# MicroYY/VoxelHashing

Hardware: AMD Instinct MI355X
Metric: depth frames/sec integrate+raycast @640x480, 4 cm voxel; HBM GB/s vs peak (higher is better)
Workload: dtype f32

## Files before the change

### include/vh_api.h

```cpp
#ifndef VH_API_H
#define VH_API_H

#include "vh_types.h"

#ifdef __cplusplus
extern "C" {
#endif

typedef void* vhStream_t;

const char* vh_version(void);
const char* vh_error_string(int code);
const char* vh_last_error_message(void);

int vh_malloc(void** devPtr, size_t bytes);
int vh_free(void* devPtr);
int vh_malloc_host(void** hostPtr, size_t bytes);
int vh_free_host(void* hostPtr);
int vh_memcpy_h2d(void* dst, const void* src, size_t bytes, vhStream_t stream);
int vh_memcpy_d2h(void* dst, const void* src, size_t bytes, vhStream_t stream);
int vh_memset(void* dst, int value, size_t bytes, vhStream_t stream);
int vh_time_next_launch(void* startEvent, void* stopEvent);
int vh_time_launch_after(uint32_t skip, void* startEvent, void* stopEvent);
int vh_stream_create(vhStream_t* out);
// ... 68 lines not shown
int vh_stream_in_device(const VhHashData* hd, const VhHashParams* hp, uint32_t n, const VhSDFBlockDesc* d_descs, const VhVoxel* d_blocks,
                        int32_t lockToken, uint32_t* d_failed, uint32_t* d_bitMask, uint32_t chunkBit, uint32_t* d_mapped, uint32_t tag,
                        vhStream_t stream);
int vh_stream_in_pass1(const VhHashData* hd, const VhHashParams* hp, uint32_t n, uint32_t heapCountPrev,
                       const VhSDFBlockDesc* d_descs, int32_t lockToken, vhStream_t stream);
int vh_stream_in_pass2(const VhHashData* hd, const VhHashParams* hp, uint32_t n, uint32_t heapCountPrev,
                       const VhSDFBlockDesc* d_descs, const VhVoxel* d_blocks, vhStream_t stream);

int vh_synth_frame(const double* h_spheres, int nSpheres, int inside, const float camToWorld[16],
                   const VhDepthCameraParams* cp, float* d_depth, float* d_color4, vhStream_t stream);
enum { VH_OP_ALLOC = 0, VH_OP_DELETE = 1, VH_OP_INSERT = 2, VH_OP_LOOKUP = 3, VH_OP_NEW_PASS = 4 };
int vh_debug_hash_ops(const VhHashData* hd, const VhHashParams* hp, const int32_t* d_ops, int32_t* d_results,
                      uint32_t n, vhStream_t stream);

int vh_debug_check_fast_math(float divisor, uint32_t modulus, uint32_t n, uint32_t seed, uint32_t* d_mismatches, vhStream_t stream);

int vh_debug_check_refined_division(uint32_t n, uint32_t seed, uint32_t* d_mismatches, vhStream_t stream);
int vh_debug_check_weighted_colour(uint32_t* d_out, vhStream_t stream);
int vh_debug_valu_probe(uint32_t mode, uint32_t wavesPerSimd, uint32_t iters, uint32_t* d_stamps, uint32_t* numWaves, vhStream_t stream);

typedef struct VhSceneRep VhSceneRep;
typedef struct VhRayCast VhRayCast;
typedef struct VhChunkGrid VhChunkGrid;

int vh_scene_rep_create(const VhHashParams* hp, const VhSceneOptions* opt, vhStream_t stream, VhSceneRep** out);
void vh_scene_rep_destroy(VhSceneRep* s);
int vh_scene_rep_integrate(VhSceneRep* s, const float rigidTransform[16], const VhDepthCameraData* cam,
                           const VhDepthCameraParams* cp, const uint32_t* d_bitMask);
int vh_scene_rep_set_last_rigid_transform_and_compactify(VhSceneRep* s, const float rigidTransform[16],
                                                         const VhDepthCameraParams* cp);
// ... 309 lines not shown
```

### voxelhashing_amd/csrc/vh_device.hpp

```cpp
#pragma once

#include <hip/hip_runtime.h>
#include <stdint.h>

#include "../../include/vh_types.h"

namespace vhd {

struct F3 { float x, y, z; };
struct I3 { int x, y, z; };

#define VHD __device__ __forceinline__

VHD float minf() { return __int_as_float((int)0xff800000u); }
VHD float pinf() { return __int_as_float((int)0x7f800000u); }

VHD F3 mk3(float x, float y, float z) { F3 r; r.x = x; r.y = y; r.z = z; return r; }
VHD I3 mki3(int x, int y, int z) { I3 r; r.x = x; r.y = y; r.z = z; return r; }
VHD float dot3(F3 a, F3 b) { return a.x * b.x + a.y * b.y + a.z * b.z; }

VHD int f2i(float v) { return __float2int_rz(v); }
VHD uint8_t f2uc(float v) { return (uint8_t)__float2int_rz(fminf(fmaxf(v, 0.0f), 255.0f)); }

VHD int signi(float v) { return (0.0f < v) - (v < 0.0f); }
// ... 477 lines not shown
    const uint32_t a = v0.cw & 0x00ffffffu, c = v1.cw & 0x00ffffffu;
    uint32_t rgb = (a | c) - (((a ^ c) >> 1) & 0x7f7f7f7fu);
    float w0 = (float)v0.weight(), w1 = (float)v1.weight();
    if (hp.m_colorIntegration != VH_COLOR_RUNNING_AVERAGE) rgb = weighted_colour(v0.cw, v1.cw, w0 + w1, 1.0f / (w0 + w1));
    out.sdf = (v0.sdf * w0 + v1.sdf * w1) / (w0 + w1);
    uint32_t w = min(hp.m_integrationWeightMax, v0.weight() + v1.weight());
    out.cw = rgb | ((w & 0xffu) << 24);
    return out;
}


constexpr int kWave = 64;
VHD uint32_t lane_id() { return threadIdx.x & (kWave - 1); }
VHD uint64_t lanemask_lt() { return (1ull << lane_id()) - 1ull; }

inline uint32_t cdiv(uint64_t a, uint64_t b) { return (uint32_t)((a + b - 1) / b); }
inline uint32_t image_tiles(uint32_t width, uint32_t height) { return cdiv(width, 8) * cdiv(height, 8); }

VHD float4 f4_scale(float a, float4 v) { return make_float4(a * v.x, a * v.y, a * v.z, a * v.w); }
VHD float4 f4_add(float4 a, float4 b) { return make_float4(a.x + b.x, a.y + b.y, a.z + b.z, a.w + b.w); }
VHD float4 f4_div(float4 a, float b) { return make_float4(a.x / b, a.y / b, a.z / b, a.w / b); }

template <class Fetch>
VHD float4 bilinear_float4_taps(float x, float y, Fetch fetch, uint32_t W, uint32_t H)
{
    const int px = (int)floorf(x), py = (int)floorf(y);
    const float alpha = x - (float)px, beta = y - (float)py;
    const float mi = minf();
    float4 s0 = make_float4(0.f, 0.f, 0.f, 0.f), s1 = s0;
    float w0 = 0.0f, w1 = 0.0f;
// ... 24 lines not shown
```

### voxelhashing_amd/csrc/vh_kernels.hip

```cpp
#include <hip/hip_runtime.h>

#include <atomic>
#include <cmath>
#include <cstdint>
#include <cstring>

#include "../../include/vh_api.h"
#include "vh_device.hpp"
#include "vh_host_util.hpp"

using namespace vhd;

#include "vh_frame_alloc.hpp"
#include "vh_frame_compactify.hpp"
#include "vh_frame_integrate.hpp"
#include "vh_frame_splat.hpp"

namespace {


struct BlockCache {
    int bx0, by0, bz0, p0;
    int bx1, by1, bz1, p1;
    bool v0, v1;
// ... 18 lines not shown
    else if (!((word >> (h & 31)) & 1u)) p = VH_FREE_ENTRY;
    else p = lookup_ptr(hd, hp, mki3(bx, by, bz));
    bc.bx1 = bc.bx0; bc.by1 = bc.by0; bc.bz1 = bc.bz0; bc.p1 = bc.p0; bc.v1 = bc.v0;
    bc.bx0 = bx; bc.by0 = by; bc.bz0 = bz; bc.p0 = p; bc.v0 = true;
    return p;
}

constexpr int kPtrUnknown = -3;

struct HashLookup {
    const VhHashData& hd;
    const VhHashParams& hp;
    HashMod hm;
    BlockCache bc;
    static constexpr bool kOffsets32 = false;
    VHD int find(int bx, int by, int bz) { return cached_lookup(hd, hp, hm, bc, bx, by, bz); }
    VHD bool first_tap(int bx, int by, int bz, int& handle)
    {
        handle = kPtrUnknown;
        return bucket_maybe_occupied(hd, hash_pos_fast(hm, mki3(bx, by, bz)));
    }
    VHD bool resolve(int, int bxa, int bya, int bza, int bxb, int byb, int bzb, uint32_t straddle, int (&p)[8])
    {
        const int p0 = find(bxa, bya, bza);
        if (p0 == VH_FREE_ENTRY) return false;
#pragma unroll
        for (int j = 0; j < 8; j++) p[j] = p0;
        if (straddle) {
            uint32_t need = 0xfeu;
#pragma unroll
// ... 16 lines not shown
            }
        }
        return true;
    }
};

constexpr uint32_t kTileSlotWords = 12;

template <uint32_t kTileTabSlots, bool OFFSETS32>
struct TileLookup {
    const int* tab;
    bool complete;
    const VhHashData& hd;
    const VhHashParams& hp;
    static constexpr bool kOffsets32 = OFFSETS32;
    VHD static uint32_t slot_of(int bx, int by, int bz)
    {
        return ((__umul24((uint32_t)bx, 0x9E3779u) + __umul24((uint32_t)by, 0x7F4A7Du) + __umul24((uint32_t)bz, 0x85EBCBu)) >> 10) & (kTileTabSlots - 1u);
    }
    VHD static int slot_find(const int* tab, int bx, int by, int bz)
    {
        uint32_t h = slot_of(bx, by, bz);
        for (;;) {
            const int4 e = *reinterpret_cast<const int4*>(&tab[h * kTileSlotWords]);
            if (e.w == VH_FREE_ENTRY) return -1;
            if ((int)(e.x == bx) & (int)(e.y == by) & (int)(e.z == bz)) return (int)h;
            h = (h + 1u) & (kTileTabSlots - 1u);
        }
    }
    VHD int find_any(int bx, int by, int bz) const
// ... 28 lines not shown
#pragma unroll 1
        for (uint32_t j = 0; j < 8u; j++) {
            const int pj = find_any((j & 1u) ? bxb : bxa, (j & 2u) ? byb : bya, (j & 4u) ? bzb : bza);
            if (pj == VH_FREE_ENTRY) return false;
#pragma unroll
            for (uint32_t k = 0; k < 8u; k++) p[k] = (k == j) ? pj : p[k];
        }
        return true;
    }
};

template <uint32_t kTileTabSlots, bool OFFSETS32>
struct TileLookupComplete {
    const int* tab;
    static constexpr bool kOffsets32 = OFFSETS32;
    VHD bool first_tap(int bx, int by, int bz, int& handle) const
    {
        handle = TileLookup<kTileTabSlots, OFFSETS32>::slot_find(tab, bx, by, bz);
        if (handle >= 0) return true;
        handle = kPtrUnknown;
        return false;
    }
    VHD bool resolve(int handle, int bxa, int bya, int bza, int, int, int, uint32_t straddle, int (&p)[8]) const
    {
        const int sl = handle >= 0 ? handle : TileLookup<kTileTabSlots, OFFSETS32>::slot_find(tab, bxa, bya, bza);
        if (sl < 0) return false;
        const int* e = &tab[(uint32_t)sl * kTileSlotWords + 3u];
        int all = 0;
#pragma unroll
        for (uint32_t j = 0; j < 8u; j++) {
// ... 191 lines not shown
{
    RayQ rq;
    rq.cam = cam; rq.dir = dir;
    rq.vs = voxel;
    rq.rvs = 1.0f / rq.vs;
    rq.halfVoxel = rq.vs / 2.0f;
    rq.camq = mk3(cam.x * rq.rvs, cam.y * rq.rvs, cam.z * rq.rvs);
    rq.dirq = mk3(dir.x * rq.rvs, dir.y * rq.rvs, dir.z * rq.rvs);
    const float Q = 1.0f + (fabsf(rq.camq.x) + fabsf(rq.camq.y) + fabsf(rq.camq.z)) +
                    tFar * (fabsf(rq.dirq.x) + fabsf(rq.dirq.y) + fabsf(rq.dirq.z));
    const float margin = Q * (16.0f / 16777216.0f);
    rq.certLim = (Q < 65536.0f) ? 0.5f - margin : -1.0f;
    return rq;
}

struct Bisected {
    float alpha;
    uint32_t color;
    bool accepted;
};
template <class LK>
VHD Bisected bisect(LK& lk, const VhHashData& hd, const RayQ& rq, float lastAlpha, float lastSdf, float t, float dist,
                    float thresSampleDist, float thresDist, uint32_t& cost)
{
    float a = lastAlpha, aDist = lastSdf, b = t, bDist = dist, c = 0.0f;
    uint32_t color = 0u;
    bool success = true;
#pragma unroll 1
    for (int i = 0; i < 3; i++) {
        cost += kCostSample;
        c = a + (aDist / (aDist - bDist)) * (b - a);
        Taps ctp;
        tap_coords(rq, c, ctp);
        float cDist = 0.0f;
        if (!trilinear<true>(hd, rq.vs, lk, kPtrUnknown, ctp, mk3(rq.cam.x + c * rq.dir.x, rq.cam.y + c * rq.dir.y, rq.cam.z + c * rq.dir.z), rq.rvs, cDist, color)) { success = false; break; }
        if (aDist * cDist > 0.0f) { a = c; aDist = cDist; }
        else { b = c; bDist = cDist; }
    }
    Bisected r;
    r.alpha = c;
    r.color = color;
    r.accepted = success && fabsf(lastSdf - dist) < thresSampleDist && fabsf(dist) < thresDist;
    return r;
}

#ifndef VH_PIPELINE_SMALL
#define VH_PIPELINE_SMALL 0
#endif

struct RayHit {
    float alpha;
    uint32_t color;
    bool hit;
// ... 29 lines not shown

    const float tSkip = depthToRayLength * tileZmin;
    float tStop = fminf(rayEnd, depthToRayLength * tileZmax);
#pragma unroll 1
    while (rcur < tSkip && rcur < rayEnd) rcur += inc;
    if (half != 0u) {
        const float tMid = depthToRayLength * zMid;
        if (half == 1u) {
            tStop = fminf(tStop, tMid);
        } else {
#pragma unroll 1
            for (;;) {
                const float nxt = rcur + inc;
                if (!(nxt < tMid) || !(nxt < rayEnd)) break;
                rcur = nxt;
            }
        }
    }

    if constexpr (PIPELINED) {
        struct Pending {
            float r;
            int skipped;
            int state;
            TapLoads L;
        };
        auto fetch = [&](float r0) -> Pending {
            Pending f;
            f.skipped = 0;
            float r = r0;
// ... 100 lines not shown
#endif
            if (ok & (lastValid != 0) & (lastSdf > 0.0f) & (dist < 0.0f)) { candidate = true; break; }
            lastSdf = ok ? dist : lastSdf;
            lastAlpha = ok ? rcur : lastAlpha;
            lastValid = ok ? 1 : 0;
            rcur += inc;
        }
        if (!candidate) break;

        float a = lastAlpha, aDist = lastSdf, b = rcur, bDist = dist, c = 0.0f;
        uint32_t color2 = 0u;
        bool success = true;
#ifdef VH_RENDER_STATS
        const long long tC0 = clock64();
#endif
#pragma unroll 1
        for (int i = 0; i < 3; i++) {
#ifdef VH_RENDER_STATS
            statTri += 1.0f;
            statIter += 1.0f / (float)__popcll(__ballot(1));
#endif
            cost += kCostSample;
            c = a + (aDist / (aDist - bDist)) * (b - a);
            Taps ctp;
            tap_coords(rq, c, ctp);
            const F3 cpos = mk3(worldCamPos.x + c * worldDir.x, worldCamPos.y + c * worldDir.y, worldCamPos.z + c * worldDir.z);
            float cDist = 0.0f;
            if (!trilinear<true>(hd, rq.vs, lk, kPtrUnknown, ctp, cpos, rq.rvs, cDist, color2)) { success = false; break; }
            if (aDist * cDist > 0.0f) { a = c; aDist = cDist; }
            else { b = c; bDist = cDist; }
        }
#ifdef VH_RENDER_STATS
        statCyc[2] += (float)(clock64() - tC0);
#endif
        if (success && fabsf(lastSdf - dist) < rp.m_thresSampleDist && fabsf(dist) < rp.m_thresDist) {
            out.hit = true;
            out.alpha = c;
            out.color = color2;
            if (GRADIENTS) {
                const F3 iso = mk3(worldCamPos.x + c * worldDir.x, worldCamPos.y + c * worldDir.y, worldCamPos.z + c * worldDir.z);
                const F3 g = gradient_for_point(hd, hp, iso);
                out.normal = mat_mul_d(rp.m_viewMatrix, mk3(-g.x, -g.y, -g.z));
            }
            break;
        }
        lastSdf = dist;
        lastAlpha = rcur;
        lastValid = 1;
        rcur += inc;
    }
}

VHD void store_ray(const VhRayCastData& rd, const VhDepthCameraParams& cp, size_t pix, uint32_t x, uint32_t y, const RayHit& r, bool gradients)
{
    const float mi = minf();
    float depth = mi;
    float4 depth4 = make_float4(mi, mi, mi, mi), normal = depth4, color = depth4;
    if (r.hit) {
        depth = r.alpha / r.depthToRayLength;
        const F3 sk = depth_to_skeleton(cp, x, y, depth);
        depth4 = make_float4(sk.x, sk.y, sk.z, 1.0f);
        color = make_float4((float)(r.color & 0xffu) / 255.f, (float)((r.color >> 8) & 0xffu) / 255.f, (float)((r.color >> 16) & 0xffu) / 255.f, 1.0f);
        if (gradients) normal = make_float4(r.normal.x, r.normal.y, r.normal.z, 1.0f);
    }
    rd.d_depth[pix] = depth;
    reinterpret_cast<float4*>(rd.d_depth4)[pix] = depth4;
    if (rd.d_normals) reinterpret_cast<float4*>(rd.d_normals)[pix] = normal;
    reinterpret_cast<float4*>(rd.d_colors)[pix] = color;
}

#ifdef VH_RENDER_STATS
#define VH_STAT_DECL const long long statT0 = clock64(); const long long statR0 = wall_clock64(); float statTri = 0.0f, statIter = 0.0f; float statCyc[3] = { 0.0f, 0.0f, 0.0f };
#define VH_STAT_ARGS , statTri, statIter, statCyc
#define VH_STAT_STORE                                                                                                                   \
    {                                                                                                                                   \
        const uint32_t hwid = __builtin_amdgcn_s_getreg((31 << 11) | 4), xcc = __builtin_amdgcn_s_getreg((31 << 11) | 20);              \
        reinterpret_cast<float4*>(rd.d_depth4)[pix] = make_float4(statCyc[0], statCyc[1], statCyc[2], 0.0f);                             \
// ... 166 lines not shown
}

template <bool GRADIENTS, uint32_t CAP, bool OFFSETS32>
VHD void render_tile(const VhHashData& hd, const VhHashParams& hp, const VhRayCastData& rd, const VhDepthCameraParams& cp, const VhRayCastParams& rp,
                     uint4* heads, const int4* lists, uint32_t cap, uint32_t* sched, uint32_t phase,
                     int (*tileTab)[2u * CAP * 12u])
{
    constexpr uint32_t kTileTabSlots = 2u * CAP;
    typedef TileLookup<kTileTabSlots, OFFSETS32> Lookup;
    typedef TileLookupComplete<kTileTabSlots, OFFSETS32> LookupComplete;
    static_assert(kTileSlotWords == 12u, "tileTab row size");
    const uint32_t lane = lane_id();
    const uint32_t W = rp.m_width, H = rp.m_height;
    const uint32_t tilesX = (W + 7) / 8, tilesY = (H + 7) / 8;
    const uint32_t nTiles = tilesX * tilesY;
    const uint32_t waveIdx = (uint32_t)__builtin_amdgcn_readfirstlane((int)(blockIdx.x * (blockDim.x / kWave) + (threadIdx.x / kWave)));
    uint32_t tile = waveIdx, half = 0u;
    if (sched && sched[0] == phase) {
        const uint2 e = reinterpret_cast<const uint2*>(sched + 4 + 4u * ((nTiles + 3u) / 4u))[waveIdx];
        tile = e.y == phase ? (e.x & 0xffffffu) : nTiles;
        half = e.y == phase ? (e.x >> 24) : 0u;
    }
    if (tile >= nTiles) return;
#if defined(VH_KNOCKOUT) && VH_KNOCKOUT == 41
    const uint32_t stamp0 = (uint32_t)__builtin_amdgcn_s_memrealtime();
    uint32_t stamp1 = 0u;
    uint4* const stampAt = reinterpret_cast<uint4*>(hd.d_hashCompactified) + (hp.m_hashNumBuckets * VH_HASH_BUCKET_SIZE) / 2u + 3u * waveIdx;
    uint32_t stampList = 0u;
#define VH_WAVE_STAMP(COST)                                                                                                                     \
    if (lane == 0) {                                                                                                                             \
        stampAt[0] = make_uint4(stamp0, stamp1, (uint32_t)__builtin_amdgcn_s_memrealtime(), tile | (half << 24));                               \
        stampAt[1] = make_uint4((COST), __builtin_amdgcn_s_getreg((31 << 11) | 4), __builtin_amdgcn_s_getreg((31 << 11) | 20), 0x57410000u | waveIdx); \
        stampAt[2] = make_uint4(stampList, 0u, 0u, 0u);                                                                                           \
    }
#else
#define VH_WAVE_STAMP(COST)
// ... 86 lines not shown
                if (lane + k * kWave < listed) {
                    const int b3[3] = { mine[k].x, mine[k].y, mine[k].z };
                    float a = vm[11], b = vm[11];
#pragma unroll
                    for (int ax = 0; ax < 3; ax++) {
                        const float lo = (float)(b3[ax] * VH_SDF_BLOCK_SIZE) * vs - growLo, hi = (float)(b3[ax] * VH_SDF_BLOCK_SIZE + VH_SDF_BLOCK_SIZE) * vs + growHi;
                        const float p = vm[8 + ax] * lo, q = vm[8 + ax] * hi;
                        a += fminf(p, q);
                        b += fmaxf(p, q);
                    }
                    const float zs = 2e-3f * fmaxf(fabsf(a), fabsf(b)) + 0.5f * vs;
                    zlo = fminf(zlo, a - zs);
                    zhi = fmaxf(zhi, b + zs);
                }
            }
#pragma unroll
            for (int off = 32; off > 0; off >>= 1) {
                zlo = fminf(zlo, __shfl_xor(zlo, off));
                zhi = fmaxf(zhi, __shfl_xor(zhi, off));
            }
            if (!complete) {
                zlo = fminf(zlo, __uint_as_float(head.x));
                zhi = fmaxf(zhi, __uint_as_float(head.y));
            }
            tileZmin = fmaxf(zlo, 0.0f);
            tileZmax = zhi;
        }
    }
    tileZmin = __int_as_float(__builtin_amdgcn_readfirstlane(__float_as_int(tileZmin)));
    tileZmax = __int_as_float(__builtin_amdgcn_readfirstlane(__float_as_int(tileZmax)));
#if defined(VH_KNOCKOUT) && VH_KNOCKOUT == 41
    stamp1 = (uint32_t)__builtin_amdgcn_s_memrealtime();
#endif
    const uint32_t tileX = (tile % tilesX) * 8, tileY = (tile / tilesX) * 8;
    VH_STAT_DECL
    RayHit out;
    out.hit = false;
    uint32_t cost = 0u;
    if (const uint32_t x = tileX + (lane & 7), y = tileY + (lane >> 3); x < W && y < H && tileZmin <= tileZmax) {
        constexpr bool kPipelined = (CAP > (uint32_t)VH_TILE_LIST_CAPACITY) || VH_PIPELINE_SMALL;
        if (complete) {
            LookupComplete lk{ tab };
            march_ray<GRADIENTS, kPipelined>(lk, hd, hp, cp, rp, x, y, tileZmin, tileZmax, half, 0.5f * (tileZmin + tileZmax), out, cost VH_STAT_ARGS);
        } else {
            Lookup lk{ tab, false, hd, hp };
            march_ray<GRADIENTS, kPipelined>(lk, hd, hp, cp, rp, x, y, tileZmin, tileZmax, half, 0.5f * (tileZmin + tileZmax), out, cost VH_STAT_ARGS);
        }
    }
#pragma unroll
    for (int off = 32; off > 0; off >>= 1) cost = max(cost, (uint32_t)__shfl_xor((int)cost, off));
    const uint32_t laneAfter = lane_id_again();
    const uint32_t x = tileX + (laneAfter & 7), y = tileY + (laneAfter >> 3);
    const bool inImage = x < W && y < H;
    const size_t pix = (size_t)y * W + x;
    if (half != 0u) {
        int* mine = tab;
        int* other = tileTab[waveInGroup ^ 1u];
        if (half == 2u) {
            mine[laneAfter * 8u + 0u] = out.hit ? 1 : 0;
            mine[laneAfter * 8u + 1u] = __float_as_int(out.alpha);
            mine[laneAfter * 8u + 2u] = (int)out.color;
            if (GRADIENTS) { mine[laneAfter * 8u + 3u] = __float_as_int(out.normal.x); mine[laneAfter * 8u + 4u] = __float_as_int(out.normal.y); mine[laneAfter * 8u + 5u] = __float_as_int(out.normal.z); }
            if (laneAfter == 0) mine[64u * 8u] = (int)cost;
        }
        __syncthreads();
        if (half == 2u) { VH_WAVE_STAMP(cost) return; }
        if (!out.hit && other[laneAfter * 8u + 0u] != 0) {
            out.hit = true;
            out.alpha = __int_as_float(other[laneAfter * 8u + 1u]);
            out.color = (uint32_t)other[laneAfter * 8u + 2u];
            if (GRADIENTS) out.normal = mk3(__int_as_float(other[laneAfter * 8u + 3u]), __int_as_float(other[laneAfter * 8u + 4u]), __int_as_float(other[laneAfter * 8u + 5u]));
        }
        cost += (uint32_t)other[64u * 8u];
        if (laneAfter == 0) heads[tile] = make_uint4(0x7f800000u, 0u, 0u, 0u);
    }
    if (inImage) {
        store_ray(rd, cp, pix, x, y, out, GRADIENTS);
        VH_STAT_STORE
    }
    VH_WAVE_STAMP(cost)
    if (sched && laneAfter == 0) sched[4 + tile] = min(cost / kCostClassWidth, kCostClasses - 1u);
}
#undef VH_WAVE_STAMP
#undef VH_STAT_DECL
#undef VH_STAT_ARGS
#undef VH_STAT_STORE

struct CoAlloc {
    VhHashData hd;
    VhHashParams hp;
    VhDepthCameraData cam;
    VhDepthCameraParams cp;
    const uint32_t* bitMask;
    uint2* packed;
    HashMod hm;
    int32_t lockToken;
    uint32_t firstGroup;
};

VHD bool co_alloc(const CoAlloc& job)
{
    if (job.firstGroup == 0u || blockIdx.x < job.firstGroup) return false;
    const uint32_t g = blockIdx.x - job.firstGroup;
    if (g == 0u && threadIdx.x == 0) job.hd.d_hashCompactifiedCounter[0] = 0;
    alloc_tile(job.hd, job.hp, job.cam, job.cp, job.bitMask, job.lockToken, job.hm, job.packed, g * (256u / kWave) + (threadIdx.x / kWave));
    return true;
}
inline uint32_t co_alloc_groups(uint32_t tiles) { return cdiv(tiles, 256u / kWave); }

#ifndef VH_RENDER_WAVES
#define VH_RENDER_WAVES 6
#endif
template <bool GRADIENTS, bool OFFSETS32>
__global__ __launch_bounds__(256) __attribute__((amdgpu_waves_per_eu(VH_RENDER_WAVES, VH_RENDER_WAVES)))
void k_render(VhHashData hd, VhHashParams hp, VhRayCastData rd, VhDepthCameraParams cp, VhRayCastParams rp,
              uint4* heads, const int4* lists, uint32_t cap, uint32_t* sched, uint32_t phase, CoAlloc job)
{
    __shared__ int tileTab[256 / kWave][2u * VH_TILE_LIST_CAPACITY * kTileSlotWords];
    if (co_alloc(job)) return;
    render_tile<GRADIENTS, VH_TILE_LIST_CAPACITY, OFFSETS32>(hd, hp, rd, cp, rp, heads, lists, cap, sched, phase, tileTab);
}

template <bool GRADIENTS, bool OFFSETS32>
__global__ __launch_bounds__(256)
void k_render_large(VhHashData hd, VhHashParams hp, VhRayCastData rd, VhDepthCameraParams cp, VhRayCastParams rp,
                    uint4* heads, const int4* lists, uint32_t cap, uint32_t* sched, uint32_t phase, CoAlloc job)
{
    __shared__ int tileTab[256 / kWave][2u * VH_TILE_LIST_CAPACITY_LARGE * kTileSlotWords];
    if (co_alloc(job)) return;
    render_tile<GRADIENTS, VH_TILE_LIST_CAPACITY_LARGE, OFFSETS32>(hd, hp, rd, cp, rp, heads, lists, cap, sched, phase, tileTab);
}

}

#include "vh_frame_normals.hpp"
#include "vh_frame_checks.hpp"


static uint32_t device_num_cus()
{
    static int numCUs = 0;
    if (numCUs == 0) {
        int dev = 0;
        if (hipGetDevice(&dev) != hipSuccess || hipDeviceGetAttribute(&numCUs, hipDeviceAttributeMultiprocessorCount, dev) != hipSuccess || numCUs <= 0)
// ... 181 lines not shown

uint32_t vh_debug_render_force_offsets64(uint32_t on) { return (uint32_t)g_forceOffsets64.exchange(on ? 1 : 0, std::memory_order_relaxed); }

int vh_render_intervals_co(const VhHashData* hd, const VhHashParams* hp, const VhRayCastData* rd, const VhDepthCameraParams* cp,
                           const VhRayCastParams* rp, uint32_t* d_tileHeads, const VhTileBlock* d_tileBlocks, uint32_t tileCapacity,
                           uint32_t* d_schedule, uint32_t phase, VhFrameJob* fj, vhStream_t stream)
{
    if (!hd || !hp || !rd || !cp || !rp || !rd->d_depth || !d_tileHeads) return VH_ERR_BAD_ARGUMENT;
    const uint32_t tiles = image_tiles(rp->m_width, rp->m_height);
    if (tiles == 0) return VH_OK;
    uint4* h = reinterpret_cast<uint4*>(d_tileHeads);
    const int4* l = reinterpret_cast<const int4*>(d_tileBlocks);
    const uint32_t cap = d_tileBlocks ? tileCapacity : 0u;
    const bool large = cap > (uint32_t)VH_TILE_LIST_CAPACITY;
    uint32_t groups = cdiv(tiles + (d_schedule ? split_tiles(tiles) : 0u), 4);
    CoAlloc job;
    std::memset(&job, 0, sizeof(job));
    if (fj && !fj->allocLaunched && fj->cam.d_depthData && fj->hashData.d_hash && fj->hashParams.m_hashNumBuckets >= 2) {
        job.hd = fj->hashData; job.hp = fj->hashParams; job.cam = fj->cam; job.cp = fj->cp;
        job.bitMask = fj->d_bitMask;
        job.packed = reinterpret_cast<uint2*>(fj->d_packedFrame);
        job.hm = make_hash_mod(fj->hashParams.m_hashNumBuckets);
        job.lockToken = fj->lockToken;
        job.firstGroup = groups;
        groups += co_alloc_groups(image_tiles(fj->cp.m_imageWidth, fj->cp.m_imageHeight));
        fj->allocLaunched = 1;
    }
    const dim3 grid(groups);
    hipStream_t st = (hipStream_t)stream;
    const bool o32 = vh_render_offsets32(hp->m_numSDFBlocks) != 0;
// ... 132 lines not shown
```

### voxelhashing_amd/csrc/vh_util.hip

```cpp
#include <hip/hip_runtime.h>

#include "../../include/vh_api.h"
#include "vh_device.hpp"
#include "vh_host_util.hpp"

using namespace vhd;

namespace {

struct SynthArgs {
    double spheres[4 * 8];
    int nSpheres;
    int inside;
    float T[16];
};

__global__ __launch_bounds__(256) void k_synth(SynthArgs a, VhDepthCameraParams cp, float* depth, float4* color)
{
    const uint32_t idx = blockIdx.x * blockDim.x + threadIdx.x;
    if (idx >= cp.m_imageWidth * cp.m_imageHeight) return;
    const uint32_t u = idx % cp.m_imageWidth, v = idx / cp.m_imageWidth;
    const double ox = (double)a.T[3], oy = (double)a.T[7], oz = (double)a.T[11];
    const double dx = ((double)u - (double)cp.mx) / (double)cp.fx;
    const double dy = ((double)v - (double)cp.my) / (double)cp.fy;
// ... 36 lines not shown
    s ^= s >> 15; s *= 2246822519u; s ^= s >> 13; s *= 3266489917u; s ^= s >> 16;
    uint32_t u = s * 747796405u + 2891336453u;
    float a;
    if ((i & 7u) == 7u) {
        a = __uint_as_float(u);
        const uint32_t ex = (u >> 23) & 0xffu;
        if (ex == 0xffu || ex < 0x10u || ex > 0xe8u) a = (float)(int)u * 1.0e-6f;
    } else {
        a = ((float)(int)u) * (1.0f / 2147483648.0f) * (((i >> 3) & 1u) ? 400.0f : 8.0f);
    }
    const float rb = 1.0f / b;
    const float q0 = a / b, q1 = div_exact(a, b, rb);
    if (__float_as_uint(q0) != __float_as_uint(q1) && !(q0 == 0.0f && q1 == 0.0f)) atomicAdd(&mismatches[0], 1u);
    if ((s % hm.d) != umod_fast(s, hm)) atomicAdd(&mismatches[1], 1u);
    if ((u % hm.d) != umod_fast(u, hm)) atomicAdd(&mismatches[1], 1u);
    if (i < 64u) {
        const uint32_t e = 0xffffffffu - i;
        if ((e % hm.d) != umod_fast(e, hm)) atomicAdd(&mismatches[1], 1u);
        if ((i % hm.d) != umod_fast(i, hm)) atomicAdd(&mismatches[1], 1u);
    }
}

}

extern "C" {

int vh_synth_frame(const double* h_spheres, int nSpheres, int inside, const float camToWorld[16],
                   const VhDepthCameraParams* cp, float* d_depth, float* d_color4, vhStream_t stream)
{
    if (!h_spheres || !camToWorld || !cp || !d_depth || !d_color4 || nSpheres < 0 || nSpheres > 8) return VH_ERR_BAD_ARGUMENT;
    SynthArgs a;
    for (int i = 0; i < 4 * nSpheres; i++) a.spheres[i] = h_spheres[i];
    a.nSpheres = nSpheres;
    a.inside = inside;
    for (int i = 0; i < 16; i++) a.T[i] = camToWorld[i];
    const uint64_t n = (uint64_t)cp->m_imageWidth * cp->m_imageHeight;
    if (n == 0) return VH_OK;
    k_synth<<<cdiv(n, 256), 256, 0, (hipStream_t)stream>>>(a, *cp, d_depth, reinterpret_cast<float4*>(d_color4));
    return vh_last_launch_error();
}

int vh_debug_check_fast_math(float divisor, uint32_t modulus, uint32_t n, uint32_t seed, uint32_t* d_mismatches, vhStream_t stream)
{
    if (!d_mismatches || modulus < 2 || !(divisor > 0.0f)) return VH_ERR_BAD_ARGUMENT;
    VH_HIP(hipMemsetAsync(d_mismatches, 0, 2 * sizeof(uint32_t), (hipStream_t)stream));
    if (n == 0) return VH_OK;
    k_check_fast_math<<<cdiv(n, 256), 256, 0, (hipStream_t)stream>>>(divisor, make_hash_mod(modulus), n, seed, d_mismatches);
    return vh_last_launch_error();
}

}
```

### voxelhashing_amd/lib.py

```python
import ctypes as C
import os

import numpy as np

from . import vhtypes as T

_HERE = os.path.dirname(os.path.abspath(__file__))
LIB_PATH = os.environ.get("VH_LIB_PATH") or os.path.join(_HERE, "libvoxelhashing_amd.so")
_LIB = None

P = C.POINTER
_F16 = P(C.c_float)
_VP = C.c_void_p

PROTOTYPES = {
    "vh_version": (C.c_char_p, []),
    "vh_error_string": (C.c_char_p, [C.c_int]),
    "vh_last_error_message": (C.c_char_p, []),
    "vh_malloc": (C.c_int, [P(_VP), C.c_size_t]),
    "vh_free": (C.c_int, [_VP]),
    "vh_malloc_host": (C.c_int, [P(_VP), C.c_size_t]),
    "vh_free_host": (C.c_int, [_VP]),
    "vh_memcpy_h2d": (C.c_int, [_VP, _VP, C.c_size_t, _VP]),
    "vh_memcpy_d2h": (C.c_int, [_VP, _VP, C.c_size_t, _VP]),
# ... 30 lines not shown
    "vh_debug_render_force_offsets64": (C.c_uint32, [C.c_uint32]),
    "vh_compute_normals": (C.c_int, [_VP, _VP, C.c_uint32, C.c_uint32, _VP]),
    "vh_render_intervals_co": (C.c_int, [P(T.HashData), P(T.HashParams), P(T.RayCastData), P(T.DepthCameraParams), P(T.RayCastParams), _VP, _VP, C.c_uint32, _VP, C.c_uint32, P(T.FrameJob), _VP]),
    "vh_compute_normals_co": (C.c_int, [_VP, _VP, C.c_uint32, C.c_uint32, P(T.FrameJob), _VP]),
    "vh_compute_normals_co2": (C.c_int, [_VP, _VP, C.c_uint32, C.c_uint32, P(T.FrameJob), P(T.RayCastParams), _VP, _VP, C.c_uint32, _VP, C.c_uint32, _VP, _VP]),
    "vh_stream_out_pass1": (C.c_int, [P(T.HashData), P(T.HashParams), C.c_uint32, C.c_uint32, C.c_float, _F16, _VP, _VP, C.c_uint32, C.c_int32, _VP]),
    "vh_stream_out_pass2": (C.c_int, [P(T.HashData), P(T.HashParams), _VP, _VP, C.c_uint32, _VP]),
    "vh_stream_out_device": (C.c_int, [P(T.HashData), P(T.HashParams), C.c_uint32, C.c_uint32, C.c_float, _F16, _VP, _VP, _VP, C.c_uint32, C.c_int32, _VP, _VP]),
    "vh_publish_count": (C.c_int, [_VP, _VP, C.c_uint32, _VP]),
    "vh_stream_in_device": (C.c_int, [P(T.HashData), P(T.HashParams), C.c_uint32, _VP, _VP, C.c_int32, _VP, _VP, C.c_uint32, _VP, C.c_uint32, _VP]),
    "vh_stream_in_pass1": (C.c_int, [P(T.HashData), P(T.HashParams), C.c_uint32, C.c_uint32, _VP, C.c_int32, _VP]),
    "vh_stream_in_pass2": (C.c_int, [P(T.HashData), P(T.HashParams), C.c_uint32, C.c_uint32, _VP, _VP, _VP]),
    "vh_synth_frame": (C.c_int, [_VP, C.c_int, C.c_int, _F16, P(T.DepthCameraParams), _VP, _VP, _VP]),
    "vh_debug_hash_ops": (C.c_int, [P(T.HashData), P(T.HashParams), _VP, _VP, C.c_uint32, _VP]),
    "vh_debug_check_fast_math": (C.c_int, [C.c_float, C.c_uint32, C.c_uint32, C.c_uint32, _VP, _VP]),
    "vh_debug_valu_probe": (C.c_int, [C.c_uint32, C.c_uint32, C.c_uint32, _VP, P(C.c_uint32), _VP]),
    "vh_debug_check_refined_division": (C.c_int, [C.c_uint32, C.c_uint32, _VP, _VP]),
    "vh_debug_check_weighted_colour": (C.c_int, [_VP, _VP]),
    "vh_publish_words": (C.c_int, [_VP, _VP, _VP, C.c_uint32, _VP]),
    "vh_stream_out_probe": (C.c_int, [_VP, _VP, C.c_uint32, C.c_uint32, C.c_float, _VP, _VP, _VP, C.c_uint32, _VP]),
    "vh_scene_rep_create": (C.c_int, [P(T.HashParams), P(T.SceneOptions), _VP, P(_VP)]),
    "vh_scene_rep_destroy": (None, [_VP]),
    "vh_scene_rep_integrate": (C.c_int, [_VP, _F16, P(T.DepthCameraData), P(T.DepthCameraParams), _VP]),
    "vh_scene_rep_set_last_rigid_transform_and_compactify": (C.c_int, [_VP, _F16, P(T.DepthCameraParams)]),
    "vh_scene_rep_reset": (C.c_int, [_VP]),
    "vh_scene_rep_get_hash_data": (C.c_int, [_VP, P(T.HashData)]),
    "vh_scene_rep_get_hash_params": (C.c_int, [_VP, P(T.HashParams)]),
    "vh_scene_rep_get_heap_free_count": (C.c_int, [_VP, P(C.c_uint32)]),
    "vh_scene_rep_get_num_occupied_blocks": (C.c_int, [_VP, P(C.c_uint32)]),
    "vh_scene_rep_debug_hash": (C.c_int, [_VP, P(C.c_uint32)]),
# ... 322 lines not shown
```

Before: 21980.

## Use DPP wave reductions, colourless bisection steps, and per-lane split-ray costs in raycast

Replaces shuffle-based wave min/max reductions with inline DPP assembly plus readlane, and skips colour fetches in the first two bisection steps when gradients are off. It also changes the split-tile cost accounting to per-lane (reducing after merging halves), adjusts the cost estimate for complete tile lookups, and replaces the colour divide with div_exact. Schedule loading now uses a single 64-bit read and falls back to the wave index when the schedule is stale, and a bounds check on the schedule buffer plus a debug reduce kernel are added. The aim is to cut shuffle/LDS traffic and memory reads in the raycast hot path. In exchange it brings in hand-written asm with hazard nops and changes the scheduling semantics.

```diff
diff --git a/include/vh_api.h b/include/vh_api.h
--- a/include/vh_api.h
+++ b/include/vh_api.h
@@ -106,6 +106,8 @@
                       uint32_t n, vhStream_t stream);
 
 int vh_debug_check_fast_math(float divisor, uint32_t modulus, uint32_t n, uint32_t seed, uint32_t* d_mismatches, vhStream_t stream);
+
+int vh_debug_wave_reduce(const uint32_t* d_in64, uint32_t* d_out192, vhStream_t stream);
 
 int vh_debug_check_refined_division(uint32_t n, uint32_t seed, uint32_t* d_mismatches, vhStream_t stream);
 int vh_debug_check_weighted_colour(uint32_t* d_out, vhStream_t stream);
diff --git a/voxelhashing_amd/csrc/vh_device.hpp b/voxelhashing_amd/csrc/vh_device.hpp
--- a/voxelhashing_amd/csrc/vh_device.hpp
+++ b/voxelhashing_amd/csrc/vh_device.hpp
@@ -515,6 +515,32 @@
 VHD uint32_t lane_id() { return threadIdx.x & (kWave - 1); }
 VHD uint64_t lanemask_lt() { return (1ull << lane_id()) - 1ull; }
 
+#define VH_WAVE_REDUCE(OP, CONSTRAINT)                                                                        \
+    {                                                                                                         \
+        asm("s_nop 1\n\t" OP " %0, %0, %0 row_shr:1 row_mask:0xf bank_mask:0xf" : CONSTRAINT(v));             \
+        asm("s_nop 1\n\t" OP " %0, %0, %0 row_shr:2 row_mask:0xf bank_mask:0xf" : CONSTRAINT(v));             \
+        asm("s_nop 1\n\t" OP " %0, %0, %0 row_shr:4 row_mask:0xf bank_mask:0xf" : CONSTRAINT(v));             \
+        asm("s_nop 1\n\t" OP " %0, %0, %0 row_shr:8 row_mask:0xf bank_mask:0xf" : CONSTRAINT(v));             \
+        asm("s_nop 1\n\t" OP " %0, %0, %0 row_bcast:15 row_mask:0xa bank_mask:0xf" : CONSTRAINT(v));          \
+        asm("s_nop 1\n\t" OP " %0, %0, %0 row_bcast:31 row_mask:0xc bank_mask:0xf" : CONSTRAINT(v));          \
+    }
+VHD float wave_min_f32(float v)
+{
+    VH_WAVE_REDUCE("v_min_f32_dpp", "+v")
+    return __int_as_float(__builtin_amdgcn_readlane(__float_as_int(v), kWave - 1));
+}
+VHD float wave_max_f32(float v)
+{
+    VH_WAVE_REDUCE("v_max_f32_dpp", "+v")
+    return __int_as_float(__builtin_amdgcn_readlane(__float_as_int(v), kWave - 1));
+}
+VHD uint32_t wave_max_u32(uint32_t v)
+{
+    VH_WAVE_REDUCE("v_max_u32_dpp", "+v")
+    return (uint32_t)__builtin_amdgcn_readlane((int)v, kWave - 1);
+}
+#undef VH_WAVE_REDUCE
+
 inline uint32_t cdiv(uint64_t a, uint64_t b) { return (uint32_t)((a + b - 1) / b); }
 inline uint32_t image_tiles(uint32_t width, uint32_t height) { return cdiv(width, 8) * cdiv(height, 8); }
 
diff --git a/voxelhashing_amd/csrc/vh_kernels.hip b/voxelhashing_amd/csrc/vh_kernels.hip
--- a/voxelhashing_amd/csrc/vh_kernels.hip
+++ b/voxelhashing_amd/csrc/vh_kernels.hip
@@ -56,6 +56,7 @@
     HashMod hm;
     BlockCache bc;
     static constexpr bool kOffsets32 = false;
+    static constexpr bool kGeneral = true;
     VHD int find(int bx, int by, int bz) { return cached_lookup(hd, hp, hm, bc, bx, by, bz); }
     VHD bool first_tap(int bx, int by, int bz, int& handle)
     {
@@ -102,6 +103,7 @@
     const VhHashData& hd;
     const VhHashParams& hp;
     static constexpr bool kOffsets32 = OFFSETS32;
+    static constexpr bool kGeneral = true;
     VHD static uint32_t slot_of(int bx, int by, int bz)
     {
         return ((__umul24((uint32_t)bx, 0x9E3779u) + __umul24((uint32_t)by, 0x7F4A7Du) + __umul24((uint32_t)bz, 0x85EBCBu)) >> 10) & (kTileTabSlots - 1u);
@@ -160,6 +162,7 @@
 struct TileLookupComplete {
     const int* tab;
     static constexpr bool kOffsets32 = OFFSETS32;
+    static constexpr bool kGeneral = false;
     VHD bool first_tap(int bx, int by, int bz, int& handle) const
     {
         handle = TileLookup<kTileTabSlots, OFFSETS32>::slot_find(tab, bx, by, bz);
@@ -381,6 +384,24 @@
     return rq;
 }
 
+#ifdef VH_RENDER_STATS
+#define VH_STAT_BISECT_SAMPLE statTri += 1.0f; statIter += 1.0f / (float)__popcll(__ballot(1));
+#else
+#define VH_STAT_BISECT_SAMPLE
+#endif
+#define VH_BISECT_STEP(COLOR, CAM, DIR, COLOUR, STAT)                                                                               \
+    {                                                                                                                               \
+        STAT                                                                                                                        \
+        cost += kCostSample;                                                                                                        \
+        c = a + (aDist / (aDist - bDist)) * (b - a);                                           \
+        Taps ctp;                                                                                                                   \
+        tap_coords(rq, c, ctp);                                                                                                     \
+        const F3 cpos = mk3((CAM).x + c * (DIR).x, (CAM).y + c * (DIR).y, (CAM).z + c * (DIR).z);                                   \
+        float cDist = 0.0f;                                                                                                         \
+        if (!trilinear<COLOR>(hd, rq.vs, lk, kPtrUnknown, ctp, cpos, rq.rvs, cDist, COLOUR)) { success = false; break; }            \
+        if (aDist * cDist > 0.0f) { a = c; aDist = cDist; }                                                                         \
+        else { b = c; bDist = cDist; }                                                                                              \
+    }
 struct Bisected {
     float alpha;
     uint32_t color;
@@ -394,16 +415,8 @@
     uint32_t color = 0u;
     bool success = true;
 #pragma unroll 1
-    for (int i = 0; i < 3; i++) {
-        cost += kCostSample;
-        c = a + (aDist / (aDist - bDist)) * (b - a);
-        Taps ctp;
-        tap_coords(rq, c, ctp);
-        float cDist = 0.0f;
-        if (!trilinear<true>(hd, rq.vs, lk, kPtrUnknown, ctp, mk3(rq.cam.x + c * rq.dir.x, rq.cam.y + c * rq.dir.y, rq.cam.z + c * rq.dir.z), rq.rvs, cDist, color)) { success = false; break; }
-        if (aDist * cDist > 0.0f) { a = c; aDist = cDist; }
-        else { b = c; bDist = cDist; }
-    }
+    for (int i = 0; i < 2; i++) VH_BISECT_STEP(false, rq.cam, rq.dir, color, )
+    if (success) do VH_BISECT_STEP(true, rq.cam, rq.dir, color, ) while (0);
     Bisected r;
     r.alpha = c;
     r.color = color;
@@ -463,6 +476,13 @@
                 const float nxt = rcur + inc;
                 if (!(nxt < tMid) || !(nxt < rayEnd)) break;
                 rcur = nxt;
+            }
+            if (!LK::kGeneral && !GRADIENTS && rcur < tMid && rcur < tStop) {
+                const F3 pd = mk3((rq.cam.x + rcur * rq.dir.x) - rq.halfVoxel, (rq.cam.y + rcur * rq.dir.y) - rq.halfVoxel, (rq.cam.z + rcur * rq.dir.z) - rq.halfVoxel);
+                int h0 = kPtrUnknown;
+                const bool there = lk.first_tap(vvp_to_block1(world_to_vvp1_rb(pd.x, rq.vs, rq.rvs)), vvp_to_block1(world_to_vvp1_rb(pd.y, rq.vs, rq.rvs)),
+                                                vvp_to_block1(world_to_vvp1_rb(pd.z, rq.vs, rq.rvs)), h0);
+                cost -= 1u + (there ? kCostSample : 0u);
             }
         }
     }
@@ -593,21 +613,13 @@
 #ifdef VH_RENDER_STATS
         const long long tC0 = clock64();
 #endif
-#pragma unroll 1
-        for (int i = 0; i < 3; i++) {
-#ifdef VH_RENDER_STATS
-            statTri += 1.0f;
-            statIter += 1.0f / (float)__popcll(__ballot(1));
-#endif
-            cost += kCostSample;
-            c = a + (aDist / (aDist - bDist)) * (b - a);
-            Taps ctp;
-            tap_coords(rq, c, ctp);
-            const F3 cpos = mk3(worldCamPos.x + c * worldDir.x, worldCamPos.y + c * worldDir.y, worldCamPos.z + c * worldDir.z);
-            float cDist = 0.0f;
-            if (!trilinear<true>(hd, rq.vs, lk, kPtrUnknown, ctp, cpos, rq.rvs, cDist, color2)) { success = false; break; }
-            if (aDist * cDist > 0.0f) { a = c; aDist = cDist; }
-            else { b = c; bDist = cDist; }
+        if constexpr (GRADIENTS) {
+#pragma unroll 1
+            for (int i = 0; i < 3; i++) VH_BISECT_STEP(true, worldCamPos, worldDir, color2, VH_STAT_BISECT_SAMPLE)
+        } else {
+#pragma unroll 1
+            for (int i = 0; i < 2; i++) VH_BISECT_STEP(false, worldCamPos, worldDir, color2, VH_STAT_BISECT_SAMPLE)
+            if (success) do VH_BISECT_STEP(true, worldCamPos, worldDir, color2, VH_STAT_BISECT_SAMPLE) while (0);
         }
 #ifdef VH_RENDER_STATS
         statCyc[2] += (float)(clock64() - tC0);
@@ -630,6 +642,9 @@
     }
 }
 
+#undef VH_BISECT_STEP
+#undef VH_STAT_BISECT_SAMPLE
+
 VHD void store_ray(const VhRayCastData& rd, const VhDepthCameraParams& cp, size_t pix, uint32_t x, uint32_t y, const RayHit& r, bool gradients)
 {
     const float mi = minf();
@@ -639,7 +654,9 @@
         depth = r.alpha / r.depthToRayLength;
         const F3 sk = depth_to_skeleton(cp, x, y, depth);
         depth4 = make_float4(sk.x, sk.y, sk.z, 1.0f);
-        color = make_float4((float)(r.color & 0xffu) / 255.f, (float)((r.color >> 8) & 0xffu) / 255.f, (float)((r.color >> 16) & 0xffu) / 255.f, 1.0f);
+        constexpr float r255 = 1.0f / 255.0f;
+        color = make_float4(div_exact((float)(r.color & 0xffu), 255.0f, r255), div_exact((float)((r.color >> 8) & 0xffu), 255.0f, r255),
+                            div_exact((float)((r.color >> 16) & 0xffu), 255.0f, r255), 1.0f);
         if (gradients) normal = make_float4(r.normal.x, r.normal.y, r.normal.z, 1.0f);
     }
     rd.d_depth[pix] = depth;
@@ -836,12 +853,15 @@
     const uint32_t W = rp.m_width, H = rp.m_height;
     const uint32_t tilesX = (W + 7) / 8, tilesY = (H + 7) / 8;
     const uint32_t nTiles = tilesX * tilesY;
-    const uint32_t waveIdx = (uint32_t)__builtin_amdgcn_readfirstlane((int)(blockIdx.x * (blockDim.x / kWave) + (threadIdx.x / kWave)));
+    const uint32_t waveIdx = (uint32_t)__builtin_amdgcn_readfirstlane((int)(blockIdx.x * (256u / kWave) + (threadIdx.x / kWave)));
     uint32_t tile = waveIdx, half = 0u;
-    if (sched && sched[0] == phase) {
-        const uint2 e = reinterpret_cast<const uint2*>(sched + 4 + 4u * ((nTiles + 3u) / 4u))[waveIdx];
-        tile = e.y == phase ? (e.x & 0xffffffu) : nTiles;
-        half = e.y == phase ? (e.x >> 24) : 0u;
+    if (sched) {
+        const uint32_t made = sched[0];
+        const unsigned long long ev = reinterpret_cast<const unsigned long long*>(sched + 4 + 4u * ((nTiles + 3u) / 4u))[waveIdx];
+        const uint2 e = make_uint2((uint32_t)ev, (uint32_t)(ev >> 32));
+        const bool fresh = made == phase, dealt = e.y == phase;
+        tile = fresh ? (dealt ? (e.x & 0xffffffu) : nTiles) : waveIdx;
+        half = fresh && dealt ? (e.x >> 24) : 0u;
     }
     if (tile >= nTiles) return;
 #if defined(VH_KNOCKOUT) && VH_KNOCKOUT == 41
@@ -958,17 +978,12 @@
                     zhi = fmaxf(zhi, b + zs);
                 }
             }
-#pragma unroll
-            for (int off = 32; off > 0; off >>= 1) {
-                zlo = fminf(zlo, __shfl_xor(zlo, off));
-                zhi = fmaxf(zhi, __shfl_xor(zhi, off));
-            }
             if (!complete) {
                 zlo = fminf(zlo, __uint_as_float(head.x));
                 zhi = fmaxf(zhi, __uint_as_float(head.y));
             }
-            tileZmin = fmaxf(zlo, 0.0f);
-            tileZmax = zhi;
+            tileZmin = wave_min_f32(fmaxf(zlo, 0.0f));
+            tileZmax = wave_max_f32(zhi);
         }
     }
     tileZmin = __int_as_float(__builtin_amdgcn_readfirstlane(__float_as_int(tileZmin)));
@@ -991,8 +1006,7 @@
             march_ray<GRADIENTS, kPipelined>(lk, hd, hp, cp, rp, x, y, tileZmin, tileZmax, half, 0.5f * (tileZmin + tileZmax), out, cost VH_STAT_ARGS);
         }
     }
-#pragma unroll
-    for (int off = 32; off > 0; off >>= 1) cost = max(cost, (uint32_t)__shfl_xor((int)cost, off));
+    if constexpr (GRADIENTS) cost = wave_max_u32(cost);
     const uint32_t laneAfter = lane_id_again();
     const uint32_t x = tileX + (laneAfter & 7), y = tileY + (laneAfter >> 3);
     const bool inImage = x < W && y < H;
@@ -1005,23 +1019,26 @@
             mine[laneAfter * 8u + 1u] = __float_as_int(out.alpha);
             mine[laneAfter * 8u + 2u] = (int)out.color;
             if (GRADIENTS) { mine[laneAfter * 8u + 3u] = __float_as_int(out.normal.x); mine[laneAfter * 8u + 4u] = __float_as_int(out.normal.y); mine[laneAfter * 8u + 5u] = __float_as_int(out.normal.z); }
-            if (laneAfter == 0) mine[64u * 8u] = (int)cost;
+            if constexpr (GRADIENTS) { if (laneAfter == 0) mine[64u * 8u] = (int)cost; }
+            else mine[laneAfter * 8u + 6u] = (int)cost;
         }
         __syncthreads();
         if (half == 2u) { VH_WAVE_STAMP(cost) return; }
+        if constexpr (!GRADIENTS) { if (!out.hit) cost += (uint32_t)other[laneAfter * 8u + 6u]; }
         if (!out.hit && other[laneAfter * 8u + 0u] != 0) {
             out.hit = true;
             out.alpha = __int_as_float(other[laneAfter * 8u + 1u]);
             out.color = (uint32_t)other[laneAfter * 8u + 2u];
             if (GRADIENTS) out.normal = mk3(__int_as_float(other[laneAfter * 8u + 3u]), __int_as_float(other[laneAfter * 8u + 4u]), __int_as_float(other[laneAfter * 8u + 5u]));
         }
-        cost += (uint32_t)other[64u * 8u];
+        if constexpr (GRADIENTS) cost += (uint32_t)other[64u * 8u];
         if (laneAfter == 0) heads[tile] = make_uint4(0x7f800000u, 0u, 0u, 0u);
     }
     if (inImage) {
         store_ray(rd, cp, pix, x, y, out, GRADIENTS);
         VH_STAT_STORE
     }
+    if constexpr (!GRADIENTS) cost = wave_max_u32(cost);
     VH_WAVE_STAMP(cost)
     if (sched && laneAfter == 0) sched[4 + tile] = min(cost / kCostClassWidth, kCostClasses - 1u);
 }
@@ -1042,15 +1059,22 @@
     uint32_t firstGroup;
 };
 
-VHD bool co_alloc(const CoAlloc& job)
-{
-    if (job.firstGroup == 0u || blockIdx.x < job.firstGroup) return false;
-    const uint32_t g = blockIdx.x - job.firstGroup;
+VHD bool co_alloc(const CoAlloc& job, uint32_t firstGroup)
+{
+    if (firstGroup == 0u || blockIdx.x < firstGroup) return false;
+    const uint32_t g = blockIdx.x - firstGroup;
     if (g == 0u && threadIdx.x == 0) job.hd.d_hashCompactifiedCounter[0] = 0;
     alloc_tile(job.hd, job.hp, job.cam, job.cp, job.bitMask, job.lockToken, job.hm, job.packed, g * (256u / kWave) + (threadIdx.x / kWave));
     return true;
 }
 inline uint32_t co_alloc_groups(uint32_t tiles) { return cdiv(tiles, 256u / kWave); }
+
+VHD uint32_t render_start(const VhRayCastParams& rp, uint4* heads, const int4* lists, uint32_t cap, uint32_t* sched, uint32_t phase, const CoAlloc& job)
+{
+    uint32_t firstGroup = job.firstGroup;
+    asm("" : "+s"(firstGroup) : "s"(rp.m_width), "s"(rp.m_height), "s"(heads), "s"(lists), "s"(cap), "s"(sched), "s"(phase));
+    return firstGroup;
+}
 
 #ifndef VH_RENDER_WAVES
 #define VH_RENDER_WAVES 6
@@ -1061,7 +1085,7 @@
               uint4* heads, const int4* lists, uint32_t cap, uint32_t* sched, uint32_t phase, CoAlloc job)
 {
     __shared__ int tileTab[256 / kWave][2u * VH_TILE_LIST_CAPACITY * kTileSlotWords];
-    if (co_alloc(job)) return;
+    if (co_alloc(job, render_start(rp, heads, lists, cap, sched, phase, job))) return;
     render_tile<GRADIENTS, VH_TILE_LIST_CAPACITY, OFFSETS32>(hd, hp, rd, cp, rp, heads, lists, cap, sched, phase, tileTab);
 }
 
@@ -1071,7 +1095,7 @@
                     uint4* heads, const int4* lists, uint32_t cap, uint32_t* sched, uint32_t phase, CoAlloc job)
 {
     __shared__ int tileTab[256 / kWave][2u * VH_TILE_LIST_CAPACITY_LARGE * kTileSlotWords];
-    if (co_alloc(job)) return;
+    if (co_alloc(job, render_start(rp, heads, lists, cap, sched, phase, job))) return;
     render_tile<GRADIENTS, VH_TILE_LIST_CAPACITY_LARGE, OFFSETS32>(hd, hp, rd, cp, rp, heads, lists, cap, sched, phase, tileTab);
 }
 
@@ -1283,6 +1307,8 @@
     const uint32_t cap = d_tileBlocks ? tileCapacity : 0u;
     const bool large = cap > (uint32_t)VH_TILE_LIST_CAPACITY;
     uint32_t groups = cdiv(tiles + (d_schedule ? split_tiles(tiles) : 0u), 4);
+    if (d_schedule && (size_t)(4u + 4u * cdiv(tiles, 4) + 2u * 4u * groups) * sizeof(uint32_t) > vh_render_schedule_bytes(rp->m_width, rp->m_height))
+        return VH_ERR_BAD_ARGUMENT;
     CoAlloc job;
     std::memset(&job, 0, sizeof(job));
     if (fj && !fj->allocLaunched && fj->cam.d_depthData && fj->hashData.d_hash && fj->hashParams.m_hashNumBuckets >= 2) {
diff --git a/voxelhashing_amd/csrc/vh_util.hip b/voxelhashing_amd/csrc/vh_util.hip
--- a/voxelhashing_amd/csrc/vh_util.hip
+++ b/voxelhashing_amd/csrc/vh_util.hip
@@ -74,11 +74,24 @@
     if (__float_as_uint(q0) != __float_as_uint(q1) && !(q0 == 0.0f && q1 == 0.0f)) atomicAdd(&mismatches[0], 1u);
     if ((s % hm.d) != umod_fast(s, hm)) atomicAdd(&mismatches[1], 1u);
     if ((u % hm.d) != umod_fast(u, hm)) atomicAdd(&mismatches[1], 1u);
+    if (i < 256u) {
+        const float c = (float)i;
+        if (__float_as_uint(c / 255.f) != __float_as_uint(div_exact(c, 255.0f, 1.0f / 255.0f))) atomicAdd(&mismatches[0], 1u);
+    }
     if (i < 64u) {
         const uint32_t e = 0xffffffffu - i;
         if ((e % hm.d) != umod_fast(e, hm)) atomicAdd(&mismatches[1], 1u);
         if ((i % hm.d) != umod_fast(i, hm)) atomicAdd(&mismatches[1], 1u);
     }
+}
+
+__global__ __launch_bounds__(64) void k_wave_reduce(const uint32_t* __restrict__ in, uint32_t* __restrict__ out)
+{
+    const uint32_t lane = lane_id();
+    const uint32_t w = in[lane];
+    out[lane] = __float_as_uint(wave_min_f32(__uint_as_float(w)));
+    out[kWave + lane] = __float_as_uint(wave_max_f32(__uint_as_float(w)));
+    out[2 * kWave + lane] = wave_max_u32(w);
 }
 
 }
@@ -109,4 +122,11 @@
     return vh_last_launch_error();
 }
 
+int vh_debug_wave_reduce(const uint32_t* d_in64, uint32_t* d_out192, vhStream_t stream)
+{
+    if (!d_in64 || !d_out192) return VH_ERR_BAD_ARGUMENT;
+    k_wave_reduce<<<1, kWave, 0, (hipStream_t)stream>>>(d_in64, d_out192);
+    return vh_last_launch_error();
 }
+
+}
diff --git a/voxelhashing_amd/lib.py b/voxelhashing_amd/lib.py
--- a/voxelhashing_amd/lib.py
+++ b/voxelhashing_amd/lib.py
@@ -68,6 +68,7 @@
     "vh_synth_frame": (C.c_int, [_VP, C.c_int, C.c_int, _F16, P(T.DepthCameraParams), _VP, _VP, _VP]),
     "vh_debug_hash_ops": (C.c_int, [P(T.HashData), P(T.HashParams), _VP, _VP, C.c_uint32, _VP]),
     "vh_debug_check_fast_math": (C.c_int, [C.c_float, C.c_uint32, C.c_uint32, C.c_uint32, _VP, _VP]),
+    "vh_debug_wave_reduce": (C.c_int, [_VP, _VP, _VP]),
     "vh_debug_valu_probe": (C.c_int, [C.c_uint32, C.c_uint32, C.c_uint32, _VP, P(C.c_uint32), _VP]),
     "vh_debug_check_refined_division": (C.c_int, [C.c_uint32, C.c_uint32, _VP, _VP]),
     "vh_debug_check_weighted_colour": (C.c_int, [_VP, _VP]),
```

After: 22240, median of 6. +1.2%, better.
